# jalhajj/mahout

Measured on AMD Instinct MI355X. Metric: sketch updates/sec + item-pair cosines/sec @1M items, 1/2/4/8 MI355X, higher is better.
Workload: dtype u32

## Files before the change

mahout_amd/csrc/cms_api.hip:

```cpp
#include <hip/hip_runtime.h>

#include <atomic>
#include <chrono>
#include <rccl/rccl.h>

#include <algorithm>
#include <thread>
#include <cmath>
#include <cstdarg>
#include <cstdio>
#include <cstdlib>
#include <cstring>
#include <new>
#include <vector>

#include "cms_internal.h"

namespace cms {

static thread_local char g_err[512] = "";

int set_error(int code, const char* fmt, ...) {
  va_list ap;
  va_start(ap, fmt);
// ... 325 lines not shown
    if (hipGetDevice(&dev) != hipSuccess) dev = 0;
  }
  h->device = dev;
  hipError_t e = hipSetDevice(dev);
  if (e != hipSuccess) {
    delete h;
    return hip_fail(e, "hipSetDevice");
  }
  {
    int cus = 0;
    if (hipDeviceGetAttribute(&cus, hipDeviceAttributeMultiprocessorCount, dev) == hipSuccess && cus > 0)
      h->num_cus = cus;
  }
  h->n = p->num_owners;
  h->dw = (int64_t)p->depth * p->width;
  java_hash_params(p->seed, h->p.depth, h->a, h->b);
  HashParams& hp = h->hp;
  std::memset(&hp, 0, sizeof(hp));
  for (int i = 0; i < h->p.depth; ++i) {
    hp.ap[i] = reduce_key(h->a[i]);
    hp.bp[i] = reduce_key(h->b[i]);
  }
  hp.width = (uint32_t)h->p.width;
  hp.depth = h->p.depth;
  hp.frac_bits = p->frac_bits;
  hash_finish(hp);
  if (per_owner) h->dw = 0;

  size_t tbytes = sizeof(uint16_t) * (size_t)h->n * (size_t)h->dw;
  if ((e = hipStreamCreateWithFlags(&h->stream, hipStreamDefault)) != hipSuccess ||
      (e = hipStreamCreateWithFlags(&h->side_stream, hipStreamNonBlocking)) != hipSuccess ||
      (e = hipStreamCreateWithFlags(&h->side_stream2, hipStreamNonBlocking)) != hipSuccess ||
      (e = hipEventCreateWithFlags(&h->ev_join3, hipEventDisableTiming)) != hipSuccess ||
      (e = hipEventCreateWithFlags(&h->ev_spans, hipEventDisableTiming)) != hipSuccess ||
      (e = hipEventCreateWithFlags(&h->ev_plan, hipEventDisableTiming)) != hipSuccess ||
      (e = hipEventCreateWithFlags(&h->ev_fork2, hipEventDisableTiming)) != hipSuccess ||
      (e = hipEventCreateWithFlags(&h->ev_join2, hipEventDisableTiming)) != hipSuccess ||
#ifdef CMS_BUILD_GATHERHASH
      (e = hipMalloc((void**)&h->hp.gtab, sizeof(uint4) << 24)) != hipSuccess ||
#endif
      (!per_owner && !f64 && (e = hipMalloc(&h->d_off, sizeof(int64_t) * h->n)) != hipSuccess) ||
      (f64 && (e = hipMalloc(&h->d_t64, 4 * tbytes)) != hipSuccess) ||
      (!per_owner && (e = hipMalloc(&h->d_hidx, sizeof(int32_t) * h->n)) != hipSuccess) ||
      (!per_owner && (e = hipMemset(h->d_hidx, 0xff, sizeof(int32_t) * h->n)) != hipSuccess) ||
      (!per_owner && !f64 && (e = hipMalloc(&h->d_cbound, sizeof(uint32_t) * h->n)) != hipSuccess) ||
      (e = hipMalloc(&h->d_row_mass, sizeof(uint64_t) * h->n)) != hipSuccess ||
      (!per_owner && (e = hipMalloc(&h->d_norm, sizeof(uint64_t) * h->n * p->depth)) != hipSuccess) ||
      (!per_owner && (e = hipMalloc(&h->d_norm_sqrt, sizeof(double) * h->n * p->depth)) != hipSuccess) ||
      (e = hipMalloc(&h->d_rowmax, sizeof(uint32_t) * h->n)) != hipSuccess ||
      (e = hipMalloc(&h->d_flags, 64 * sizeof(uint32_t))) != hipSuccess ||
      (e = hipHostMalloc((void**)&h->h_pin, 16 * sizeof(uint32_t), hipHostMallocDefault)) != hipSuccess ||
      (e = hipMemset(h->d_flags, 0, 64 * sizeof(uint32_t))) != hipSuccess ||
      (e = hipMemset(h->d_row_mass, 0, sizeof(uint64_t) * h->n)) != hipSuccess) {
    int rc = hip_fail(e, "cms_create allocation");
    cms_destroy(h);
    return rc;
  }
  h->empty = true;
  h->norms_valid = false;
  h->forms_ok = !per_owner && !f64 && h->p.width % 32 == 0 && h->tune.forms;
  h->compact = h->forms_ok && !h->tune.no_compact &&
               (double)h->n * (double)(slot_units(h->dw) / kRowAlign + 1) < 4.0e9;
  if (!per_owner && !f64) {
    if (int rc = init_row_offsets(h)) {
      cms_destroy(h);
      return rc;
    }
  }
  *out = h;
  return CMS_OK;
}

int cms_create(const cms_params* p, cms_handle** out) { return create_impl(p, false, out); }

int cms_create_per_owner(const cms_params* p, cms_handle** out) { return create_impl(p, true, out); }

void cms_destroy(cms_handle* h) {
  if (!h) return;
  (void)hipSetDevice(h->device);
  if (h->stream) (void)hipStreamSynchronize(h->stream);
  for (auto& pe : h->pending) {
    (void)hipEventDestroy(pe.start);
    (void)hipEventDestroy(pe.stop);
  }
  for (hipEvent_t e : h->event_pool) (void)hipEventDestroy(e);
  if (h->order_ev) (void)hipEventDestroy(h->order_ev);
  if (h->side_stream) (void)hipStreamSynchronize(h->side_stream);
  if (h->side_stream2) (void)hipStreamSynchronize(h->side_stream2);
  if (h->ev_join3) (void)hipEventDestroy(h->ev_join3);
  if (h->ev_spans) (void)hipEventDestroy(h->ev_spans);
  if (h->ev_plan) (void)hipEventDestroy(h->ev_plan);
  if (h->ev_fork2) (void)hipEventDestroy(h->ev_fork2);
  if (h->ev_join2) (void)hipEventDestroy(h->ev_join2);
  free_query_pool(h);
  if (h->comm) (void)ncclCommDestroy(h->comm);
  arena_release(h);
  void* bufs[] = {h->d_off, h->d_t64, h->d_hidx, h->d_cbound, h->d_row_mass, h->d_norm, h->d_norm_sqrt, h->d_rowmax, h->d_flags, h->d_owner_ids};
  for (void* b : bufs)
    if (b) (void)hipFree(b);
  if (h->h_pin) (void)hipHostFree(h->h_pin);
  DevBuf* ws[] = {&h->ws_in_row, &h->ws_in_key, &h->ws_in_val, &h->ws_p1_row, &h->ws_p1_key, &h->ws_p1_val,
                  &h->ws_csr_key, &h->ws_csr_val, &h->ws_csr_off, &h->ws_csr_hi, &h->ws_hotpart, &h->ws_hist, &h->ws_small, &h->ws_partials,
                  &h->ws_hot, &h->ws_query, &h->ws_out, &h->ws_limb0, &h->ws_limbmeta, &h->ws_limbhot,
                  &h->ws_hotlist, &h->ws_tiles, &h->ws_slab, &h->ws_topq, &h->vl[0].buf, &h->vl[1].buf, &h->ws_nsq, &h->ws_cand,
                  &h->dlog_row, &h->dlog_key, &h->dlog_val, &h->dlog_cnt, &h->dlog_all, &h->ws_srow,
                  &h->ws_f4, &h->ws_i8blk, &h->po_off, &h->po_kp, &h->po_inc, &h->po_shape, &h->po_sk, &h->po_norm, &h->po_nsq,
                  &h->po_scratch, &h->po_wrows, &h->po_s0, &h->ws_pothr, &h->ws_posurv, &h->hot_tab, &h->ws_bound, &h->ws_force, &h->ws_plist, &h->ws_blist,
                  &h->ws_mbnd, &h->ws_mbits, &h->ws_mwoff, &h->ws_mpacked, &h->rf_ids, &h->rf_sc, &h->rf_cnt,
                  &h->rf_full, &h->rf_touch, &h->rf_new, &h->rf_redo, &h->rf_perm};
  for (DevBuf* b : ws) b->release();
  if (h->stream) (void)hipStreamDestroy(h->stream);
  if (h->side_stream) (void)hipStreamDestroy(h->side_stream);
  if (h->side_stream2) (void)hipStreamDestroy(h->side_stream2);
  delete h;
}

int cms_set_owner_ids(cms_handle* h, const int64_t* ids, int64_t n) {
  if (!h || !ids) return set_error(CMS_E_PARAM, "null argument");
  Guard g(h);
  if (n != h->n) return set_error(CMS_E_PARAM, "expected %lld owner IDs, got %lld", (long long)h->n, (long long)n);
  for (int64_t i = 1; i < n; ++i)
    if (ids[i] <= ids[i - 1]) return set_error(CMS_E_PARAM, "owner IDs must be strictly ascending");
// ... 1291 lines not shown
```

mahout_amd/csrc/cms_build.hip:

```cpp
#include <hip/hip_runtime.h>

#include <algorithm>
#include <cstdlib>

#include "cms_device.h"
#include "cms_internal.h"

namespace cms {

#ifdef CMS_BUILD_CHEAPHASH
#define bucket(hp, d, kp) ((uint32_t)(((kp) >> (d)) & (hp).wmask))
#endif
#ifdef CMS_BUILD_GATHERHASH
#define bucket(hp, d, kp) \
  ((uint32_t)(((&(hp).gtab[(kp) & 0xFFFFFFu].x)[((d) >> 1) & 3] >> (((d) & 1) << 4)) & (hp).wmask))
#endif

struct HotInfo {
  int64_t row;
  int32_t nslices;
  int32_t e0;
};

constexpr int kKeyRegs = 4;
// ... 388 lines not shown
    lds_barrier();
    d += two ? 2 : 1;
  }
  }

  if (badv) atomicOr(flags, kFlagBadValue);
  mass = wave_sum_u64_sat(mass);
  if ((tid & 63) == 0 && mass) atomicAdd(&s_mass, (unsigned long long)mass);
#pragma unroll
  for (int o = 32; o > 0; o >>= 1) vmax = max(vmax, (uint32_t)__shfl_xor((int)vmax, o, 64));
  if ((tid & 63) == 0 && vmax) atomicMax(&s_max, vmax);
  __syncthreads();
  if (!atomic_mode && tid < hp.depth) norm[row * hp.depth + tid] = s_norm[tid];
  if (!atomic_mode && tid == 0) rowmax[row] = s_max;
  if (tid == 0) {
    uint64_t tm = s_mass;
    if (!atomic_mode) {
      uint64_t m = accumulate ? row_mass[row] + tm : tm;
      row_mass[row] = m;
      if (m >= (1ULL << 32)) atomicOr(flags, kFlagOverflow);
    } else if (tm) {
      unsigned long long old = atomicAdd((unsigned long long*)&row_mass[row], (unsigned long long)tm);
      if (old + tm >= (1ULL << 32)) atomicOr(flags, kFlagOverflow);
    }
  }
}

constexpr int kMidThreads = 256;
constexpr int64_t kMidCachedKeys = (int64_t)kMidThreads * kKeyRegs;
constexpr int64_t kStreamBigKeys = 4096;
__device__ __forceinline__ int32_t list2_at(const int32_t* list, uint32_t cap, uint32_t nfront, uint32_t i) {
  return i < nfront ? list[i] : list[cap - 1u - (i - nfront)];
}
enum { kCntSlot = 0, kCntMid = 1 , kCntStream = 3 , kCntTicket = 5, kCntWords = 8 };
constexpr int kClassChunk = 4096;
__global__ __launch_bounds__(256) void k_build_classes(const int64_t* lo_, const int64_t* hi_, int64_t nrows,
                                                       const int32_t* hidx, const uint64_t* bound, int32_t* slot_list,
                                                       int32_t* mid_list, int32_t* stream_list, uint32_t* cnt) {
  __shared__ int32_t s_own[kClassChunk], s_str[kClassChunk];
  __shared__ uint32_t s_n[4], s_b[4];
  const int lane = (int)__lane_id();
  const int tid = threadIdx.x;
  const uint32_t cap = (uint32_t)nrows;
  const unsigned long long below = (1ULL << lane) - 1ULL;
  for (int64_t r0 = (int64_t)blockIdx.x * kClassChunk; r0 < nrows; r0 += (int64_t)gridDim.x * kClassChunk) {
    if (tid < 4) s_n[tid] = 0;
    __syncthreads();
    for (int64_t r = r0 + tid; r < r0 + kClassChunk; r += 256) {
      bool is[4] = {false, false, false, false};
      if (r < nrows) {
        const int32_t sl = hidx[r];
        const int64_t m = hi_[r] - lo_[r];
        is[0] = sl >= 0;
        const bool is_mid = !is[0] && !byte_class(sl, m, bound[r]);
        is[1] = is_mid && m <= kMidCachedKeys;
        is[2] = is_mid && m > kStreamBigKeys;
        is[3] = is_mid && !is[1] && !is[2];
      }
      unsigned long long mk[4];
      uint32_t b[4] = {0, 0, 0, 0};
#pragma unroll
      for (int k = 0; k < 4; ++k) {
        mk[k] = __ballot(is[k]);
        if (lane == 0 && mk[k]) b[k] = atomicAdd(&s_n[k], (uint32_t)__popcll(mk[k]));
        b[k] = (uint32_t)__shfl((int)b[k], 0, 64) + (uint32_t)__popcll(mk[k] & below);
      }
      if (is[0]) s_own[b[0]] = (int32_t)r;
      if (is[1]) s_own[kClassChunk - 1 - b[1]] = (int32_t)r;
      if (is[2]) s_str[b[2]] = (int32_t)r;
      if (is[3]) s_str[kClassChunk - 1 - b[3]] = (int32_t)r;
    }
    __syncthreads();
    if (tid < 4) {
      const int ci = tid == 0 ? kCntSlot : tid == 1 ? kCntMid + 1 : kCntStream + tid - 2;
      s_b[tid] = s_n[tid] ? atomicAdd(&cnt[ci], s_n[tid]) : 0u;
    }
    __syncthreads();
    for (uint32_t i = tid; i < s_n[0]; i += 256) slot_list[s_b[0] + i] = s_own[i];
    for (uint32_t i = tid; i < s_n[1]; i += 256) mid_list[cap - 1u - (s_b[1] + i)] = s_own[kClassChunk - 1 - i];
    for (uint32_t i = tid; i < s_n[2]; i += 256) stream_list[s_b[2] + i] = s_str[i];
    for (uint32_t i = tid; i < s_n[3]; i += 256) stream_list[cap - 1u - (s_b[3] + i)] = s_str[kClassChunk - 1 - i];
    __syncthreads();
  }
}

constexpr int kMidListKeys = kBuildThreads * kKeyRegs;
constexpr int kMidRowKeys = 4;
template <int SV, int D, int MT>
__device__ __forceinline__ void mid_rows(
    const int64_t* lo_, const int64_t* hi_, const Keys& keys, const float* vals, const HashParams& hp,
    const int32_t* list, const uint32_t* list_cnt, uint32_t cap, const TableView& tv, int32_t* hidx_w,
    uint32_t* cbound, uint64_t* row_mass, uint64_t* norm, uint32_t* rowmax, uint32_t* flags, int list_keys,
    int u4_keys, int u8_keys) {
  static_assert(MT == kMidThreads, "one instantiation per depth");
  constexpr int MTH = MT;
  constexpr int MKR = kKeyRegs;
  extern __shared__ __align__(16) uint32_t lds[];
  __shared__ unsigned long long s_norm[CMS_MAX_DEPTH];
  __shared__ unsigned long long s_mass;
  __shared__ uint32_t s_max, s_ovf;
  const int tid = threadIdx.x;
  const int w = (int)hp.width;
  const uint32_t nfront = list_cnt[0], count = nfront + list_cnt[1];
  for (uint32_t li = blockIdx.x; li < count; li += gridDim.x) {
    const int64_t row = list2_at(list, cap, nfront, li);
    const int64_t lo = lo_[row], hi = hi_[row];
    const bool cached = (hi - lo) <= (int64_t)MTH * MKR;
    uint64_t kp[MKR];
    uint32_t ik[MKR];
    uint64_t mass = 0;
    bool badv = false;
    if (cached) {
#pragma unroll
      for (int k = 0; k < MKR; ++k) {
        const int64_t i = lo + tid + (int64_t)k * MTH;
        kp[k] = 0;
        ik[k] = 0;
        if (i < hi) {
          uint32_t inc;
          if (!load_inc(vals, i, inc, hp.frac_bits)) {
            badv = true;
            inc = 0;
          }
          kp[k] = keys.at(i);
          ik[k] = inc;
          mass += inc;
        }
      }
    }
    uint4* d4 = reinterpret_cast<uint4*>(tv.row16(row));
    const int64_t m = hi - lo;
    const bool as_list = cached && m <= list_keys && vals == nullptr && hp.frac_bits == 0 &&
                         (int64_t)hp.depth * m <= 8192 && 2 + 2 * (int64_t)hp.depth * m < (int64_t)hp.depth * w / 2;
    uint16_t* lst = tv.row16(row);
    int level = -1;
    uint32_t vmax = 0;
    const int start = as_list || m <= u4_keys ? 0 : m <= u8_keys ? 1 : 2;
    bool mass_pending = !cached;
    if (start == 0) {
      constexpr int ab = 4;
      const int lga = 3;
      const uint32_t capa = (1u << ab) - 1u;
      const int nq_all = (int)((int64_t)hp.depth * w * ab >> 7);
      uint4* l4 = reinterpret_cast<uint4*>(lds);
      for (int j = tid; j < nq_all; j += MTH) l4[j] = make_uint4(0, 0, 0, 0);
      if (tid < CMS_MAX_DEPTH) s_norm[tid] = 0ULL;
      if (tid == 0) {
        s_max = 0u;
        s_ovf = 0u;
        s_mass = 0ULL;
      }
      __syncthreads();
      bool ovf = false;
      vmax = 0;
      constexpr int kSq = D > 0 ? D : 1;
      uint32_t sqr[kSq];
#pragma unroll
      for (int d = 0; d < kSq; ++d) sqr[d] = 0u;
      const bool tele = D > 0 && as_list;
      auto add_all = [&](uint64_t kr, uint32_t inc, int64_t lt) {
        each_bucket<D>(hp, kr, [&](int d, uint32_t bk) {
          if (lt >= 0) lst[1 + (int64_t)d * m + lt] = (uint16_t)bk;
          const uint32_t c = (uint32_t)d * (uint32_t)w + bk;
          const uint32_t sh = (c & ((1u << lga) - 1u)) * (uint32_t)ab;
          const uint32_t old = (atomicAdd(&lds[c >> lga], inc << sh) >> sh) & capa;
          const uint32_t nv = old + inc;
          ovf |= nv > capa || inc > capa;
          vmax = max(vmax, nv);
          if (D > 0) sqr[D > 0 ? d : 0] += (2u * old + inc) * inc;
        });
// ... 280 lines not shown
      if (tid < depth) {
        uint64_t s = 0;
#pragma unroll
        for (int k = 0; k < NW; ++k) s += red[k * RS + tid];
        norm[row * depth + tid] = s;
      }
      if (tid == 0) {
        rowmax[row] = mx;
        row_mass[row] = (uint64_t)m;
        hidx_w[row] = kFormU8;
        cbound[row] = mx;
      }
    }
    li = lds[0];
  }
}

template <int SV, int D, int MT>
__global__ __launch_bounds__(MT) __attribute__((amdgpu_waves_per_eu(MT == kStreamThreads ? 8 : 4, 8))) void k_build_mid(
    const int64_t* lo_, const int64_t* hi_, Keys keys, const float* vals, HashParams hp,
    const int32_t* list, const uint32_t* list_cnt , uint32_t cap, TableView tv, int32_t* hidx_w,
    uint32_t* cbound, uint64_t* row_mass, uint64_t* norm, uint32_t* rowmax, uint32_t* flags, int list_keys,
    int u4_keys, int u8_keys, int32_t* redo, uint32_t* redo_cnt, uint32_t* ticket) {
  if constexpr (MT == kStreamThreads)
    mid_streamed<SV, D>(lo_, hi_, keys, hp, list, list_cnt, cap, tv, hidx_w, cbound, row_mass, norm, rowmax, redo,
                        redo_cnt, ticket, u4_keys, u8_keys);
  else
    mid_rows<SV, D, MT>(lo_, hi_, keys, vals, hp, list, list_cnt, cap, tv, hidx_w, cbound, row_mass, norm, rowmax,
                        flags, list_keys, u4_keys, u8_keys);
}

constexpr int kMidGridPerCu = 8;
constexpr int kNibWaves = 4;
__host__ __device__ __forceinline__ int nib_first_bits(int64_t m, int w, int bit_keys, int crumb_keys) {
  return (m <= bit_keys && (w & 127) == 0) ? 1 : (m <= crumb_keys && (w & 63) == 0) ? 2 : 4;
}
__host__ __device__ __forceinline__ bool nib_list_row(int64_t m, int w, int d, bool weighted, int frac_bits,
                                                      int bit_keys, int crumb_keys, int list_keys) {
  return m <= list_keys && !weighted && frac_bits == 0 &&
         2 + 2 * (int64_t)d * m <= ((int64_t)d * w * nib_first_bits(m, w, bit_keys, crumb_keys)) / 8;
}

__global__ void k_row_caps(const int64_t* lo_, const int64_t* hi_, int64_t n, const uint64_t* bound,
                           const int32_t* hidx, int forms, int weighted, int frac_bits, int d, int w, int bit_keys,
                           int crumb_keys, int list_keys, uint32_t* caps) {
  const int64_t dw = (int64_t)d * w;
  const uint32_t full = (uint32_t)(slot_units(dw) / kRowAlign);
  for (int64_t r = blockIdx.x * (int64_t)blockDim.x + threadIdx.x; r < n; r += (int64_t)gridDim.x * blockDim.x) {
    const int32_t s = hidx[r];
    const int64_t m = hi_[r] - lo_[r];
    uint32_t c = full;
    if (s >= 0) {
      c = 0;
    } else if (forms && byte_class(s, m, bound[r])) {
      const int64_t u16s = nib_list_row(m, w, d, weighted != 0, frac_bits, bit_keys, crumb_keys, list_keys)
                               ? 1 + (int64_t)d * m
                               : dw / 2;
      c = (uint32_t)((u16s + kRowAlign - 1) / kRowAlign);
    }
    caps[r] = c;
  }
}

template <int SV>
__device__ __forceinline__ void nib_owner(
    int64_t row, uint32_t* lds, const int64_t* lo_, const int64_t* hi_, const Keys& keys, const float* vals,
    const HashParams& hp, const int32_t* row_hot, const uint64_t* bound, const TableView& tv, int32_t* hidx_w,
    uint32_t* cbound, uint64_t* row_mass, uint64_t* norm, uint32_t* rowmax, uint32_t* flags, int32_t* redo,
    uint32_t* redo_cnt, int bit_keys, int crumb_keys, int list_keys, int lists_done) {
  const int lane = threadIdx.x & 63;
  const int wv = threadIdx.x >> 6;
  const int64_t lo = lo_[row], hi = hi_[row];
  if (row_hot[row] >= 0 || !byte_class(tv.hidx[row], hi - lo, bound[row])) return;
  const int w = (int)hp.width;
// ... 233 lines not shown
      const int ns = (m + 63) >> 6;
      const bool ovf = ns == 1   ? list_rows<D, 1>(slot, pk, lane, m, sq, vmax)
                       : ns == 2 ? list_rows<D, 2>(slot, pk, lane, m, sq, vmax)
                       : ns == 3 ? list_rows<D, 3>(slot, pk, lane, m, sq, vmax)
                       : ns == 4 ? list_rows<D, 4>(slot, pk, lane, m, sq, vmax)
                                 : false;
      if (lane == 0) lst[0] = (uint16_t)m;
      if (ovf) {
        if (lane == 0) redo[atomicAdd(redo_cnt, 1u)] = ~(int32_t)row;
      } else {
#pragma unroll
        for (int q = 0; q < P; ++q) sq[q] = wave_fold_dpp(sq[q], [](uint32_t a, uint32_t b) { return a + b; });
        vmax = wave_fold_dpp(vmax, [](uint32_t a, uint32_t b) { return max(a, b); });
        if (lane < D) {
          uint32_t s = 0;
#pragma unroll
          for (int r = 0; r < D; ++r)
            if (lane == r) s = (sq[r >> 1] >> ((r & 1) << 4)) & 0xFFFFu;
          norm[row * D + lane] = s;
        }
        if (lane == 0) {
          rowmax[row] = vmax;
          row_mass[row] = (uint64_t)m;
          hidx_w[row] = kFormList;
          cbound[row] = vmax;
        }
      }
    }
    if (!more) break;
    row = nrow;
    lo = nlo;
    m = nm;
    raw0 = nraw0;
  }
}

template <int SV>
__global__ __launch_bounds__(kBuildThreads) void k_build_bytes(
    const int64_t* lo_, const int64_t* hi_, Keys keys, const float* vals, HashParams hp,
    const int32_t* list, const uint32_t* list_cnt, TableView tv, int32_t* hidx_w, uint32_t* cbound,
    uint64_t* row_mass, uint64_t* norm, uint32_t* rowmax, uint32_t* flags) {
  extern __shared__ __align__(16) uint32_t lds[];
  __shared__ unsigned long long s_norm[CMS_MAX_DEPTH];
  __shared__ uint32_t s_max, s_mass;
  const int tid = threadIdx.x;
  const int w = (int)hp.width;
  const int64_t dw = (int64_t)hp.depth * w;
  const uint32_t count = *list_cnt;
  for (uint32_t li = blockIdx.x; li < count; li += gridDim.x) {
    const bool keep_list = list[li] < 0;
    const int64_t row = keep_list ? ~(int64_t)list[li] : (int64_t)list[li];
    const int64_t lo = lo_[row], hi = hi_[row];
    uint16_t* lst = tv.row16(row);
    if (tid < CMS_MAX_DEPTH) s_norm[tid] = 0ULL;
    if (tid == 0) {
      s_max = 0u;
      s_mass = 0u;
    }
    uint64_t kp[kKeyRegs];
    uint32_t ik[kKeyRegs];
    uint32_t mass = 0;
    bool badv = false;
#pragma unroll
    for (int k = 0; k < kKeyRegs; ++k) {
      const int64_t i = lo + tid + (int64_t)k * kBuildThreads;
      kp[k] = 0;
// ... 301 lines not shown
  bool hot_norms_done = false;
  auto launch_hot_norms = [&]() -> int {
    TimedScope ts(h, "hot_norms");
    dim3 grid((unsigned)std::max<int64_t>(1, std::min<int64_t>(max_hot, 1024)), (unsigned)h->p.depth);
    hipLaunchKernelGGL(k_hot_norms, grid, dim3(256), 0, h->stream, hot, counters, h->hp, h->tview(), h->d_norm,
                       h->d_rowmax, whole_slices);
    CMS_HIP(hipGetLastError());
    hot_norms_done = true;
    return CMS_OK;
  };
  {
    TimedScope ts(h, "build_rows");
    auto kern = k_build_rows<kBuildStoreForm>;
    auto launch_slices = [&]() -> int {
      if (!fast_slices) return CMS_OK;
#ifdef CMS_BUILD_SKIP_SLICES
      return CMS_OK;
#endif
      static bool attr = [] {
        for (const void* f : {(const void*)k_build_slices<0>, (const void*)k_build_slices<4>,
                              (const void*)k_build_slices<5>})
          (void)hipFuncSetAttribute(f, hipFuncAttributeMaxDynamicSharedMemorySize, 80 * 1024);
        return true;
      }();
      (void)attr;
      auto kslices = h->p.depth == 5 ? k_build_slices<5> : h->p.depth == 4 ? k_build_slices<4> : k_build_slices<0>;
      hipLaunchKernelGGL(kslices, dim3((unsigned)emax), dim3(kSliceThreads), img_lds, h->stream, d_lo, d_hi,
                         keys, h->hp, kSliceKeys, hot, extra_map, counters, h->tview(), h->d_row_mass, h->d_flags,
                         whole_slices, h->d_norm, h->d_rowmax);
      CMS_HIP(hipGetLastError());
      return CMS_OK;
    };
    if (forms) {
      CMS_HIP(h->ws_blist.ensure(sizeof(int32_t) * (size_t)(3 * n + kCntWords)));
      int32_t* slot_list = h->ws_blist.as<int32_t>();
      int32_t* mid_list = slot_list + n;
      int32_t* stream_list = mid_list + n;
      uint32_t* lcnt = reinterpret_cast<uint32_t*>(stream_list + n);
      CMS_HIP(h->ws_plist.ensure(sizeof(int32_t) * (size_t)(n + 1)));
      int32_t* redo = h->ws_plist.as<int32_t>();
      uint32_t* redo_cnt = reinterpret_cast<uint32_t*>(redo + n);
      CMS_HIP(hipMemsetAsync(lcnt, 0, kCntWords * sizeof(uint32_t), h->stream));
      CMS_HIP(hipMemsetAsync(redo_cnt, 0, sizeof(uint32_t), h->stream));
      hipLaunchKernelGGL(k_build_classes,
                         dim3((unsigned)std::max<int64_t>(1, std::min<int64_t>((n + kClassChunk - 1) / kClassChunk, 1024))),
                         dim3(256), 0, h->stream, d_lo, d_hi, n, h->d_hidx, h->ws_bound.as<uint64_t>(), slot_list,
                         mid_list, stream_list, lcnt);
      CMS_HIP(hipGetLastError());
      if (h->plan_side_active) return set_error(CMS_E_STATE, "internal: side stream used while swapped for the plan");
      hipStream_t side = h->side_stream ? h->side_stream : h->stream;
#ifdef CMS_BUILD_SERIAL
      side = h->stream;
#endif
      const hipStream_t side2 = side != h->stream && h->tune.build_streams >= 3 ? h->side_stream2 : side;
      struct SideJoin {
        cms_handle* h;
        hipStream_t side, side2;
        bool armed = false;
        ~SideJoin() {
          if (armed && hipEventRecord(h->ev_join2, side) == hipSuccess)
            (void)hipStreamWaitEvent(h->stream, h->ev_join2, 0);
          if (armed && side2 != side && hipEventRecord(h->ev_join3, side2) == hipSuccess)
            (void)hipStreamWaitEvent(h->stream, h->ev_join3, 0);
        }
      } join{h, side, side2};
      if (side != h->stream) {
        CMS_HIP(hipEventRecord(h->ev_fork2, h->stream));
        CMS_HIP(hipStreamWaitEvent(side, h->ev_fork2, 0));
        if (side2 != side) CMS_HIP(hipStreamWaitEvent(side2, h->ev_fork2, 0));
        join.armed = true;
      }
      const int64_t nib_blocks = (n + kNibWaves - 1) / kNibWaves;
      const size_t nib_lds = (size_t)kNibWaves * (size_t)h->p.width / 2;
#if defined(CMS_BUILD_CHEAPHASH) || defined(CMS_BUILD_GATHERHASH)
      const int lists_done = 0;
#else
      const int lists_done = !d_val && h->hp.frac_bits == 0 && h->hp.fastq && lists_allowed(h) &&
                                     (h->p.depth == 4 || h->p.depth == 5)
                                 ? 1
                                 : 0;
#endif
      if (lists_done) {
        auto klists = h->p.depth == 5 ? k_build_lists<kBuildStoreForm, 5> : k_build_lists<kBuildStoreForm, 4>;
        if (h->lists_wgs_per_cu <= 0) {
          int per_cu = 0;
          CMS_HIP(hipOccupancyMaxActiveBlocksPerMultiprocessor(&per_cu, klists, 64 * kNibWaves, nib_lds));
          h->lists_wgs_per_cu = std::max(1, per_cu);
        }
        const int64_t lists_blocks = std::min<int64_t>(nib_blocks, (int64_t)h->num_cus * h->lists_wgs_per_cu);
        hipLaunchKernelGGL(klists, dim3((unsigned)lists_blocks), dim3(64 * kNibWaves), nib_lds, side, d_lo, d_hi, keys,
                           n, h->hp, row_hot, h->ws_bound.as<uint64_t>(), h->tview(), h->d_hidx, h->d_cbound,
                           h->d_row_mass, h->d_norm, h->d_rowmax, redo, redo_cnt, h->tune.bit_keys,
                           h->tune.crumb_keys, h->tune.list_keys);
      }
      bool nibbles_idle = lists_done != 0;
      for (int64_t m = 0; nibbles_idle && m < kByteKeys; ++m)
        nibbles_idle = nib_list_row(m, h->p.width, h->p.depth, false, 0, h->tune.bit_keys, h->tune.crumb_keys,
                                    h->tune.list_keys);
      if (!nibbles_idle)
        hipLaunchKernelGGL((k_build_nibbles<kBuildStoreForm, 0>), dim3((unsigned)nib_blocks), dim3(64 * kNibWaves),
                           nib_lds, side, d_lo, d_hi, keys, d_val, n, h->hp, row_hot, h->ws_bound.as<uint64_t>(),
                           h->tview(), h->d_hidx, h->d_cbound, h->d_row_mass, h->d_norm, h->d_rowmax, h->d_flags,
                           redo, redo_cnt, h->tune.bit_keys, h->tune.crumb_keys,
                           lists_allowed(h) ? h->tune.list_keys : 0, lists_done);
      const size_t mid_lds = std::max<size_t>((size_t)h->p.width * 2, (size_t)h->dw / 2);
      auto kmid = h->p.depth == 5   ? k_build_mid<kBuildStoreForm, 5, kMidThreads>
                  : h->p.depth == 4 ? k_build_mid<kBuildStoreForm, 4, kMidThreads>
                                    : k_build_mid<kBuildStoreForm, 0, kMidThreads>;
      auto launch_mid = [&](auto kern, int threads, unsigned grid, size_t klds, const int32_t* list, uint32_t* cnt) {
        hipLaunchKernelGGL(kern, dim3(grid), dim3(threads), klds, side2, d_lo, d_hi, keys, d_val, h->hp, list,
                           (const uint32_t*)cnt, (uint32_t)n, h->tview(), h->d_hidx, h->d_cbound, h->d_row_mass,
                           h->d_norm, h->d_rowmax, h->d_flags, lists_allowed(h) ? kMidListKeys : 0,
                           h->tune.mid_u4_keys, h->tune.mid_u8_keys, mid_list, lcnt + kCntMid, lcnt + kCntTicket);
      };
      const unsigned mid_grid = (unsigned)std::min<int64_t>(n, (int64_t)h->num_cus * kMidGridPerCu);
      bool one_pass = !d_val && h->hp.frac_bits == 0;
#ifdef CMS_BUILD_NO_STREAMED
      one_pass = false;
#endif
      if (one_pass) {
        auto kstr = h->p.depth == 5   ? k_build_mid<kBuildStoreForm, 5, kStreamThreads>
                    : h->p.depth == 4 ? k_build_mid<kBuildStoreForm, 4, kStreamThreads>
                                      : k_build_mid<kBuildStoreForm, 0, kStreamThreads>;
        const size_t str_lds = std::max<size_t>((size_t)h->dw, sizeof(uint32_t) * kStreamRedWords);
        if (h->stream_wgs_per_cu <= 0) {
          int per_cu = 0;
          CMS_HIP(hipOccupancyMaxActiveBlocksPerMultiprocessor(&per_cu, kstr, kStreamThreads, str_lds));
          h->stream_wgs_per_cu = std::max(1, per_cu);
        }
        launch_mid(kstr, kStreamThreads, (unsigned)std::min<int64_t>(n, (int64_t)h->num_cus * h->stream_wgs_per_cu),
                   str_lds, stream_list, lcnt + kCntStream);
      } else {
        launch_mid(kmid, kMidThreads, mid_grid, mid_lds, stream_list, lcnt + kCntStream);
      }
      launch_mid(kmid, kMidThreads, mid_grid, mid_lds, mid_list, lcnt + kCntMid);
      hipLaunchKernelGGL(k_build_bytes<kBuildStoreForm>, dim3((unsigned)std::min<int64_t>(n, (int64_t)h->num_cus * 2)),
                         dim3(kBuildThreads), (size_t)h->dw, side, d_lo, d_hi, keys, d_val, h->hp, redo, redo_cnt,
                         h->tview(), h->d_hidx, h->d_cbound, h->d_row_mass, h->d_norm, h->d_rowmax, h->d_flags);
      CMS_HIP(hipGetLastError());
      if ((rc0 = launch_slices())) return rc0;
      const int64_t nslot = std::min<int64_t>(n, h->hot_used);
      hipLaunchKernelGGL(kern, dim3((unsigned)(row_emax + nslot)), dim3(kBuildThreads), lds, h->stream, d_lo, d_hi,
                         keys, d_val, n, h->hp, kSliceKeys, row_hot, hot, extra_map, counters, row_emax, h->tview(),
                         h->d_row_mass, h->d_norm, h->d_rowmax, h->d_flags, accumulate, slices_done,
                         h->ws_bound.as<uint64_t>(), forms, skip_untouched, h->d_hidx, h->d_cbound,
                         (const int32_t*)slot_list, (const uint32_t*)lcnt);
      CMS_HIP(hipGetLastError());
      if (join.armed) {
        join.armed = false;
        CMS_HIP(hipEventRecord(h->ev_join2, side));
        CMS_HIP(hipStreamWaitEvent(h->stream, h->ev_join2, 0));
        if (side2 != side) {
          CMS_HIP(hipEventRecord(h->ev_join3, side2));
          CMS_HIP(hipStreamWaitEvent(h->stream, h->ev_join3, 0));
        }
      }
    } else {
      if ((rc0 = launch_slices())) return rc0;
      hipLaunchKernelGGL(kern, dim3((unsigned)(row_emax + n)), dim3(kBuildThreads), lds, h->stream, d_lo, d_hi, keys,
                         d_val, n, h->hp, kSliceKeys, row_hot, hot, extra_map, counters, row_emax, h->tview(),
                         h->d_row_mass, h->d_norm, h->d_rowmax, h->d_flags, accumulate, slices_done,
                         h->ws_bound.as<uint64_t>(), forms, skip_untouched, h->d_hidx, h->d_cbound,
                         (const int32_t*)nullptr, (const uint32_t*)nullptr);
      CMS_HIP(hipGetLastError());
    }
  }
  if (!hot_norms_done && (rc0 = launch_hot_norms())) return rc0;
// ... 7 lines not shown
```

mahout_amd/csrc/cms_internal.h:

```cpp
#pragma once
#include <hip/hip_runtime.h>
#include <rccl/rccl.h>

#include <functional>
#include <map>
#include <mutex>
#include <shared_mutex>
#include <string>
#include <vector>

#include "../../include/mahout_cms.h"
#include "cms_forms.h"
#include "cms_hash.h"

namespace cms {

enum : uint32_t {
  kFlagBadRow = 1u << 0,
  kFlagBadValue = 1u << 1,
  kFlagOverflow = 1u << 2,
};

struct DevBuf {
  void* ptr = nullptr;
// ... 125 lines not shown
}

namespace cms {
struct Tunables {
  int bit_keys = 64;
  int crumb_keys = 256;
  int list_keys = 256;
  int mid_u4_keys = 768;
  int mid_u8_keys = 12288;
  int plan_side = 1;
  int build_streams = 3;
  int po_dense_x4 = 4;
  int po_bound_part2 = 1;
  int po_bound_rows = 1;
  int po_no_prune = 0;
  int po_no_bigq = 0;
  int split_keys = 0;
  bool forms = true;
  bool no_compact = false;
  bool no_vmm = false;
  bool hot_routing = true;
  bool fp4 = true;
  bool mls = true;
};
}

struct cms_handle {
  cms_params p{};
  cms::Tunables tune;
  int device = 0;
  int num_cus = 256;
  int stream_wgs_per_cu = 0;
  int lists_wgs_per_cu = 0;
  hipStream_t stream = nullptr;
  hipStream_t side_stream = nullptr;
  hipEvent_t ev_fork2 = nullptr, ev_join2 = nullptr;
  hipStream_t side_stream2 = nullptr;
  hipEvent_t ev_join3 = nullptr;
  hipEvent_t ev_spans = nullptr, ev_plan = nullptr;
  bool spans_event = false, plan_side_request = false;
  bool plan_side_active = false;
  std::shared_mutex mu;
  std::mutex pool_mu;
  std::vector<cms::QueryCtx*> qpool;

  int64_t a[CMS_MAX_DEPTH] = {};
  int64_t b[CMS_MAX_DEPTH] = {};
  cms::HashParams hp{};

  int64_t n = 0;
  int64_t dw = 0;
  uint16_t* d_t16 = nullptr;
  int64_t t16_cap = 0, t16_used = 0;
  int64_t* d_off = nullptr;
  struct ArenaChunk {
    hipMemGenericAllocationHandle_t mem;
    size_t bytes;
  };
  void* arena_va = nullptr;
  size_t arena_va_bytes = 0, arena_mapped = 0, arena_gran = 0;
  int arena_small_layouts = 0;
  std::vector<ArenaChunk> arena_chunks;
  bool compact = false;
  bool f64 = false;
  double* d_t64 = nullptr;
  int32_t* d_hidx = nullptr;
  uint32_t* d_cbound = nullptr;
  bool forms_ok = false;
  cms::DevBuf hot_tab;
  cms::DevBuf ws_bound, ws_force, ws_plist;
  cms::DevBuf ws_blist;
// ... 308 lines not shown
```

Baseline: 55.67 billion.

## Route cached mid rows eligible for list form to a dedicated wave-per-row kernel

Adds a fifth class to the row classifier that picks cached mid rows qualifying for the compact list form. These rows go to a new k_build_mid_lists kernel on the side stream, which hashes keys in registers, counts collisions through a per-wave LDS slot array and writes list entries plus norms directly. Rows that overflow are pushed back onto the mid list for the generic path, with an event added so the later mid launch waits for them. The aim is to take the list-eligible rows off the heavier generic mid kernel, at the cost of an extra launch, a cross-stream dependency and more classifier LDS.

```diff
diff --git a/mahout_amd/csrc/cms_api.hip b/mahout_amd/csrc/cms_api.hip
--- a/mahout_amd/csrc/cms_api.hip
+++ b/mahout_amd/csrc/cms_api.hip
@@ -381,6 +381,7 @@
       (e = hipStreamCreateWithFlags(&h->side_stream, hipStreamNonBlocking)) != hipSuccess ||
       (e = hipStreamCreateWithFlags(&h->side_stream2, hipStreamNonBlocking)) != hipSuccess ||
       (e = hipEventCreateWithFlags(&h->ev_join3, hipEventDisableTiming)) != hipSuccess ||
+      (e = hipEventCreateWithFlags(&h->ev_mid_lists, hipEventDisableTiming)) != hipSuccess ||
       (e = hipEventCreateWithFlags(&h->ev_spans, hipEventDisableTiming)) != hipSuccess ||
       (e = hipEventCreateWithFlags(&h->ev_plan, hipEventDisableTiming)) != hipSuccess ||
       (e = hipEventCreateWithFlags(&h->ev_fork2, hipEventDisableTiming)) != hipSuccess ||
@@ -437,6 +438,7 @@
   if (h->side_stream) (void)hipStreamSynchronize(h->side_stream);
   if (h->side_stream2) (void)hipStreamSynchronize(h->side_stream2);
   if (h->ev_join3) (void)hipEventDestroy(h->ev_join3);
+  if (h->ev_mid_lists) (void)hipEventDestroy(h->ev_mid_lists);
   if (h->ev_spans) (void)hipEventDestroy(h->ev_spans);
   if (h->ev_plan) (void)hipEventDestroy(h->ev_plan);
   if (h->ev_fork2) (void)hipEventDestroy(h->ev_fork2);
diff --git a/mahout_amd/csrc/cms_build.hip b/mahout_amd/csrc/cms_build.hip
--- a/mahout_amd/csrc/cms_build.hip
+++ b/mahout_amd/csrc/cms_build.hip
@@ -444,35 +444,58 @@
 __device__ __forceinline__ int32_t list2_at(const int32_t* list, uint32_t cap, uint32_t nfront, uint32_t i) {
   return i < nfront ? list[i] : list[cap - 1u - (i - nfront)];
 }
-enum { kCntSlot = 0, kCntMid = 1 , kCntStream = 3 , kCntTicket = 5, kCntWords = 8 };
+__host__ __device__ __forceinline__ int nib_first_bits(int64_t m, int w, int bit_keys, int crumb_keys) {
+  return (m <= bit_keys && (w & 127) == 0) ? 1 : (m <= crumb_keys && (w & 63) == 0) ? 2 : 4;
+}
+__host__ __device__ __forceinline__ bool nib_list_row(int64_t m, int w, int d, bool weighted, int frac_bits,
+                                                      int bit_keys, int crumb_keys, int list_keys) {
+  return m <= list_keys && !weighted && frac_bits == 0 &&
+         2 + 2 * (int64_t)d * m <= ((int64_t)d * w * nib_first_bits(m, w, bit_keys, crumb_keys)) / 8;
+}
+__host__ __device__ __forceinline__ bool mid_list_row(int64_t m, int w, int d, bool weighted, int frac_bits,
+                                                      int list_keys) {
+  return m <= list_keys && !weighted && frac_bits == 0 && (int64_t)d * m <= 8192 &&
+         2 + 2 * (int64_t)d * m < (int64_t)d * w / 2;
+}
+enum {
+  kCntSlot = 0,
+  kCntMid = 1 ,
+  kCntStream = 3 ,
+  kCntTicket = 5,
+  kCntMidLists = 6,
+  kCntWords = 8
+};
 constexpr int kClassChunk = 4096;
 __global__ __launch_bounds__(256) void k_build_classes(const int64_t* lo_, const int64_t* hi_, int64_t nrows,
                                                        const int32_t* hidx, const uint64_t* bound, int32_t* slot_list,
-                                                       int32_t* mid_list, int32_t* stream_list, uint32_t* cnt) {
-  __shared__ int32_t s_own[kClassChunk], s_str[kClassChunk];
-  __shared__ uint32_t s_n[4], s_b[4];
+                                                       int32_t* mid_list, int32_t* stream_list, uint32_t* cnt,
+                                                       int32_t* mid_lists, int mid_lists_keys, int d, int w) {
+  __shared__ int32_t s_own[kClassChunk], s_str[kClassChunk], s_lst[kClassChunk];
+  __shared__ uint32_t s_n[5], s_b[5];
   const int lane = (int)__lane_id();
   const int tid = threadIdx.x;
   const uint32_t cap = (uint32_t)nrows;
   const unsigned long long below = (1ULL << lane) - 1ULL;
   for (int64_t r0 = (int64_t)blockIdx.x * kClassChunk; r0 < nrows; r0 += (int64_t)gridDim.x * kClassChunk) {
-    if (tid < 4) s_n[tid] = 0;
+    if (tid < 5) s_n[tid] = 0;
     __syncthreads();
     for (int64_t r = r0 + tid; r < r0 + kClassChunk; r += 256) {
-      bool is[4] = {false, false, false, false};
+      bool is[5] = {false, false, false, false, false};
       if (r < nrows) {
         const int32_t sl = hidx[r];
         const int64_t m = hi_[r] - lo_[r];
         is[0] = sl >= 0;
         const bool is_mid = !is[0] && !byte_class(sl, m, bound[r]);
-        is[1] = is_mid && m <= kMidCachedKeys;
+        const bool cached = is_mid && m <= kMidCachedKeys;
+        is[4] = cached && mid_list_row(m, w, d, false, 0, mid_lists_keys);
+        is[1] = cached && !is[4];
         is[2] = is_mid && m > kStreamBigKeys;
-        is[3] = is_mid && !is[1] && !is[2];
-      }
-      unsigned long long mk[4];
-      uint32_t b[4] = {0, 0, 0, 0};
-#pragma unroll
-      for (int k = 0; k < 4; ++k) {
+        is[3] = is_mid && !cached && !is[2];
+      }
+      unsigned long long mk[5];
+      uint32_t b[5] = {0, 0, 0, 0, 0};
+#pragma unroll
+      for (int k = 0; k < 5; ++k) {
         mk[k] = __ballot(is[k]);
         if (lane == 0 && mk[k]) b[k] = atomicAdd(&s_n[k], (uint32_t)__popcll(mk[k]));
         b[k] = (uint32_t)__shfl((int)b[k], 0, 64) + (uint32_t)__popcll(mk[k] & below);
@@ -481,10 +504,11 @@
       if (is[1]) s_own[kClassChunk - 1 - b[1]] = (int32_t)r;
       if (is[2]) s_str[b[2]] = (int32_t)r;
       if (is[3]) s_str[kClassChunk - 1 - b[3]] = (int32_t)r;
+      if (is[4]) s_lst[b[4]] = (int32_t)r;
     }
     __syncthreads();
-    if (tid < 4) {
-      const int ci = tid == 0 ? kCntSlot : tid == 1 ? kCntMid + 1 : kCntStream + tid - 2;
+    if (tid < 5) {
+      const int ci = tid == 0 ? kCntSlot : tid == 1 ? kCntMid + 1 : tid == 4 ? kCntMidLists : kCntStream + tid - 2;
       s_b[tid] = s_n[tid] ? atomicAdd(&cnt[ci], s_n[tid]) : 0u;
     }
     __syncthreads();
@@ -492,6 +516,7 @@
     for (uint32_t i = tid; i < s_n[1]; i += 256) mid_list[cap - 1u - (s_b[1] + i)] = s_own[kClassChunk - 1 - i];
     for (uint32_t i = tid; i < s_n[2]; i += 256) stream_list[s_b[2] + i] = s_str[i];
     for (uint32_t i = tid; i < s_n[3]; i += 256) stream_list[cap - 1u - (s_b[3] + i)] = s_str[kClassChunk - 1 - i];
+    for (uint32_t i = tid; i < s_n[4]; i += 256) mid_lists[s_b[4] + i] = s_lst[i];
     __syncthreads();
   }
 }
@@ -542,12 +567,11 @@
     }
     uint4* d4 = reinterpret_cast<uint4*>(tv.row16(row));
     const int64_t m = hi - lo;
-    const bool as_list = cached && m <= list_keys && vals == nullptr && hp.frac_bits == 0 &&
-                         (int64_t)hp.depth * m <= 8192 && 2 + 2 * (int64_t)hp.depth * m < (int64_t)hp.depth * w / 2;
+    const bool as_list = cached && mid_list_row(m, w, hp.depth, vals != nullptr, hp.frac_bits, list_keys);
     uint16_t* lst = tv.row16(row);
     int level = -1;
     uint32_t vmax = 0;
-    const int start = as_list || m <= u4_keys ? 0 : m <= u8_keys ? 1 : 2;
+    const int start = cached && li < nfront ? 2 : as_list || m <= u4_keys ? 0 : m <= u8_keys ? 1 : 2;
     bool mass_pending = !cached;
     if (start == 0) {
       constexpr int ab = 4;
@@ -894,14 +918,6 @@
 
 constexpr int kMidGridPerCu = 8;
 constexpr int kNibWaves = 4;
-__host__ __device__ __forceinline__ int nib_first_bits(int64_t m, int w, int bit_keys, int crumb_keys) {
-  return (m <= bit_keys && (w & 127) == 0) ? 1 : (m <= crumb_keys && (w & 63) == 0) ? 2 : 4;
-}
-__host__ __device__ __forceinline__ bool nib_list_row(int64_t m, int w, int d, bool weighted, int frac_bits,
-                                                      int bit_keys, int crumb_keys, int list_keys) {
-  return m <= list_keys && !weighted && frac_bits == 0 &&
-         2 + 2 * (int64_t)d * m <= ((int64_t)d * w * nib_first_bits(m, w, bit_keys, crumb_keys)) / 8;
-}
 
 __global__ void k_row_caps(const int64_t* lo_, const int64_t* hi_, int64_t n, const uint64_t* bound,
                            const int32_t* hidx, int forms, int weighted, int frac_bits, int d, int w, int bit_keys,
@@ -1201,6 +1217,195 @@
     lo = nlo;
     m = nm;
     raw0 = nraw0;
+  }
+}
+
+constexpr int kMidListWaves = 4;
+constexpr int kMidListSlots = 16;
+constexpr int kMidListGroup = 4;
+constexpr int kMidListSlotMax = 8192;
+static_assert(64 * kMidListSlots == kMidListKeys && kMidListSlots % kMidListGroup == 0, "every cached list row fits");
+
+template <int D>
+__device__ __forceinline__ bool mid_list_rows(uint32_t* slot, const uint32_t (&pk)[kMidListSlots][(D + 1) / 2],
+                                              uint32_t live, int ns, uint32_t (&sq)[D], uint32_t& vmax) {
+  bool ovf = false;
+#pragma unroll
+  for (int r = 0; r < D; ++r) {
+    uint32_t old[kMidListSlots];
+#pragma unroll
+    for (int k = 0; k < kMidListSlots; ++k)
+      if (k < ns) {
+        const uint32_t c = (pk[k][r >> 1] >> ((r & 1) << 4)) & 0xFFFFu;
+        old[k] = atomicAdd(&slot[c >> 2], ((live >> k) & 1u) << ((c & 3u) << 3));
+      }
+#pragma unroll
+    for (int k = 0; k < kMidListSlots; ++k)
+      if (k < ns) {
+        uint32_t p = pk[k][r >> 1];
+        asm volatile("" : "+v"(p));
+        const uint32_t c = (p >> ((r & 1) << 4)) & 0xFFFFu;
+        const uint32_t lv = (live >> k) & 1u;
+        const uint32_t o = (old[k] >> ((c & 3u) << 3)) & 255u;
+        const uint32_t nv = (o + 1u) * lv;
+        ovf |= nv > 255u;
+        sq[r] += (2u * o + 1u) * lv;
+        vmax = max(vmax, nv);
+        slot[c >> 2] = 0u;
+      }
+    if (__ballot(ovf)) return true;
+  }
+  return false;
+}
+
+template <int SV, int D>
+__global__ __launch_bounds__(64 * kMidListWaves) __attribute__((amdgpu_waves_per_eu(4, 8))) void k_build_mid_lists(
+    const int64_t* lo_, const int64_t* hi_, Keys keys, HashParams hp, const int32_t* list, const uint32_t* list_cnt,
+    TableView tv, int32_t* hidx_w, uint32_t* cbound, uint64_t* row_mass, uint64_t* norm, uint32_t* rowmax,
+    int32_t* redo, uint32_t* redo_cnt) {
+  extern __shared__ __align__(16) uint32_t lds[];
+  constexpr int P = (D + 1) / 2;
+  constexpr int NSL = kMidListSlots, GS = kMidListGroup, NGR = NSL / GS;
+  const int lane = threadIdx.x & 63;
+  const int wv = __builtin_amdgcn_readfirstlane(threadIdx.x >> 6);
+  const int w = (int)hp.width;
+  uint32_t* slot = lds + wv * (w >> 2);
+  for (int j = lane; j < (w >> 2); j += 64) slot[j] = 0u;
+  const uint32_t count = list_cnt[0];
+  const uint32_t idle = ((4u * (uint32_t)lane) & hp.wmask) * 0x10001u;
+  double qa[D], qb[D];
+  uint32_t am[D], bm[D];
+#pragma unroll
+  for (int r = 0; r < D; ++r) {
+    qa[r] = hp.qa[r];
+    qb[r] = hp.qb[r];
+    am[r] = (uint32_t)hp.ap[r] & hp.wmask;
+    bm[r] = (uint32_t)hp.bp[r];
+  }
+  const uint32_t stride = gridDim.x * kMidListWaves;
+  const uint32_t li = blockIdx.x * kMidListWaves + wv;
+  if (li >= count) return;
+  int32_t row = list[li];
+  int32_t row1 = li + stride < count ? list[li + stride] : -1;
+  uint32_t li2 = li + 2u * stride;
+  int64_t lo = lo_[row];
+  int m = (int)(hi_[row] - lo);
+  int64_t base = tv.base(row);
+  uint64_t raw0 = lane < m ? keys.raw(lo + lane) : 0ULL;
+  for (;;) {
+    const int32_t row2 = li2 < count ? list[li2] : -1;
+    li2 += stride;
+    int64_t nlo = 0, nhi = 0, nbase = 0;
+    if (row1 >= 0) {
+      nlo = lo_[row1];
+      nhi = hi_[row1];
+      nbase = tv.base(row1);
+    }
+    uint16_t* lst = tv.t16 + base;
+    uint32_t pk[NSL][P];
+    {
+      uint64_t cur[GS], nxt[GS];
+      cur[0] = raw0;
+#pragma unroll
+      for (int j = 1; j < GS; ++j) cur[j] = lane + 64 * j < m ? keys.raw(lo + lane + 64 * j) : 0ULL;
+#pragma unroll
+      for (int g = 0; g < NGR; ++g) {
+#pragma unroll
+        for (int j = 0; j < GS; ++j) nxt[j] = 0ULL;
+        if (g + 1 < NGR && 64 * GS * (g + 1) < m) {
+#pragma unroll
+          for (int j = 0; j < GS; ++j) {
+            const int t = lane + 64 * (GS * (g + 1) + j);
+            if (t < m) nxt[j] = keys.raw(lo + t);
+          }
+        }
+#pragma unroll
+        for (int j = 0; j < GS; ++j)
+#pragma unroll
+          for (int q = 0; q < P; ++q) pk[GS * g + j][q] = idle;
+        if (64 * GS * g < m) {
+#pragma unroll
+          for (int j = 0; j < GS; ++j) {
+            const int k = GS * g + j;
+            if (lane + 64 * k < m) {
+              uint16_t* e = lst + 1 + lane + 64 * k;
+              const uint64_t kp = keys.resolve(cur[j]);
+              const double kf = (double)(uint32_t)kp;
+              const uint32_t km = (uint32_t)kp & hp.wmask;
+              bool redo_key = (kp >> 32) != 0;
+#pragma unroll
+              for (int q = 0; q < P; ++q) pk[k][q] = 0u;
+#pragma unroll
+              for (int r = 0; r < D; ++r) {
+                const double y = fma(qa[r], kf, qb[r]);
+                const double fl = floor(y);
+                const double fr = y - fl;
+                redo_key |= !(fr >= kQEps && fr <= 1.0 - kQEps);
+                const uint32_t q = (uint32_t)__double_as_longlong(fl + 4503599627370496.0);
+                const uint32_t c = (__umul24(am[r], km) + bm[r] + __umul24(q, 25u)) & hp.wmask;
+                e[r * m] = (uint16_t)c;
+                pk[k][r >> 1] |= c << ((r & 1) << 4);
+              }
+              if (redo_key) {
+#pragma unroll 1
+                for (int r = 0; r < D; ++r) {
+                  const uint32_t c = bucket(hp, r, kp);
+                  e[r * m] = (uint16_t)c;
+#pragma unroll
+                  for (int q = 0; q < P; ++q)
+                    if ((r >> 1) == q)
+                      pk[k][q] = (r & 1) ? (pk[k][q] & 0xFFFFu) | (c << 16) : (pk[k][q] & 0xFFFF0000u) | c;
+                }
+              }
+            }
+          }
+        }
+#pragma unroll
+        for (int j = 0; j < GS; ++j) cur[j] = nxt[j];
+      }
+    }
+    int nm = 0;
+    uint64_t nraw0 = 0ULL;
+    if (row1 >= 0) {
+      nm = (int)(nhi - nlo);
+      if (lane < nm) nraw0 = keys.raw(nlo + lane);
+    }
+    uint32_t sq[D];
+#pragma unroll
+    for (int r = 0; r < D; ++r) sq[r] = 0u;
+    uint32_t vmax = 0;
+    const int nf = min(max((m - lane + 63) >> 6, 0), NSL);
+    const uint32_t live = (1u << nf) - 1u;
+    const int ns = (m + 63) >> 6;
+    const bool ovf = mid_list_rows<D>(slot, pk, live, ns, sq, vmax);
+    if (ovf) {
+      if (lane == 0) redo[atomicAdd(redo_cnt, 1u)] = row;
+    } else {
+#pragma unroll
+      for (int r = 0; r < D; ++r) sq[r] = wave_fold_dpp(sq[r], [](uint32_t a, uint32_t b) { return a + b; });
+      vmax = wave_fold_dpp(vmax, [](uint32_t a, uint32_t b) { return max(a, b); });
+      if (lane < D) {
+        uint32_t s = 0;
+#pragma unroll
+        for (int r = 0; r < D; ++r)
+          if (lane == r) s = sq[r];
+        norm[(int64_t)row * D + lane] = s;
+      }
+      if (lane == 0) {
+        lst[0] = (uint16_t)m;
+        rowmax[row] = vmax;
+        row_mass[row] = (uint64_t)m;
+        hidx_w[row] = kFormList;
+        cbound[row] = vmax;
+      }
+    }
+    if (row1 < 0) break;
+    row = row1;
+    lo = nlo;
+    m = nm;
+    base = nbase;
+    raw0 = nraw0;
+    row1 = row2;
   }
 }
 
@@ -1568,20 +1773,31 @@
       return CMS_OK;
     };
     if (forms) {
-      CMS_HIP(h->ws_blist.ensure(sizeof(int32_t) * (size_t)(3 * n + kCntWords)));
+      CMS_HIP(h->ws_blist.ensure(sizeof(int32_t) * (size_t)(4 * n + kCntWords)));
       int32_t* slot_list = h->ws_blist.as<int32_t>();
       int32_t* mid_list = slot_list + n;
       int32_t* stream_list = mid_list + n;
-      uint32_t* lcnt = reinterpret_cast<uint32_t*>(stream_list + n);
+      int32_t* mid_lists = stream_list + n;
+      uint32_t* lcnt = reinterpret_cast<uint32_t*>(mid_lists + n);
       CMS_HIP(h->ws_plist.ensure(sizeof(int32_t) * (size_t)(n + 1)));
       int32_t* redo = h->ws_plist.as<int32_t>();
       uint32_t* redo_cnt = reinterpret_cast<uint32_t*>(redo + n);
+#if defined(CMS_BUILD_CHEAPHASH) || defined(CMS_BUILD_GATHERHASH)
+      const int lists_done = 0;
+#else
+      const int lists_done = !d_val && h->hp.frac_bits == 0 && h->hp.fastq && lists_allowed(h) &&
+                                     (h->p.depth == 4 || h->p.depth == 5)
+                                 ? 1
+                                 : 0;
+#endif
+      const bool mid_lists_done = lists_done && h->p.width <= kMidListSlotMax;
       CMS_HIP(hipMemsetAsync(lcnt, 0, kCntWords * sizeof(uint32_t), h->stream));
       CMS_HIP(hipMemsetAsync(redo_cnt, 0, sizeof(uint32_t), h->stream));
       hipLaunchKernelGGL(k_build_classes,
                          dim3((unsigned)std::max<int64_t>(1, std::min<int64_t>((n + kClassChunk - 1) / kClassChunk, 1024))),
                          dim3(256), 0, h->stream, d_lo, d_hi, n, h->d_hidx, h->ws_bound.as<uint64_t>(), slot_list,
-                         mid_list, stream_list, lcnt);
+                         mid_list, stream_list, lcnt, mid_lists, mid_lists_done ? kMidListKeys : 0, h->p.depth,
+                         h->p.width);
       CMS_HIP(hipGetLastError());
       if (h->plan_side_active) return set_error(CMS_E_STATE, "internal: side stream used while swapped for the plan");
       hipStream_t side = h->side_stream ? h->side_stream : h->stream;
@@ -1608,14 +1824,22 @@
       }
       const int64_t nib_blocks = (n + kNibWaves - 1) / kNibWaves;
       const size_t nib_lds = (size_t)kNibWaves * (size_t)h->p.width / 2;
-#if defined(CMS_BUILD_CHEAPHASH) || defined(CMS_BUILD_GATHERHASH)
-      const int lists_done = 0;
-#else
-      const int lists_done = !d_val && h->hp.frac_bits == 0 && h->hp.fastq && lists_allowed(h) &&
-                                     (h->p.depth == 4 || h->p.depth == 5)
-                                 ? 1
-                                 : 0;
-#endif
+      if (mid_lists_done) {
+        auto kml = h->p.depth == 5 ? k_build_mid_lists<kBuildStoreForm, 5> : k_build_mid_lists<kBuildStoreForm, 4>;
+        const size_t ml_lds = (size_t)kMidListWaves * (size_t)h->p.width;
+        if (h->mid_lists_wgs_per_cu <= 0) {
+          int per_cu = 0;
+          CMS_HIP(hipOccupancyMaxActiveBlocksPerMultiprocessor(&per_cu, kml, 64 * kMidListWaves, ml_lds));
+          h->mid_lists_wgs_per_cu = std::max(1, per_cu);
+        }
+        const int64_t ml_blocks = std::min<int64_t>((n + kMidListWaves - 1) / kMidListWaves,
+                                                    (int64_t)h->num_cus * h->mid_lists_wgs_per_cu);
+        hipLaunchKernelGGL(kml, dim3((unsigned)ml_blocks), dim3(64 * kMidListWaves), ml_lds, side, d_lo, d_hi, keys,
+                           h->hp, (const int32_t*)mid_lists, (const uint32_t*)(lcnt + kCntMidLists), h->tview(),
+                           h->d_hidx, h->d_cbound, h->d_row_mass, h->d_norm, h->d_rowmax, mid_list, lcnt + kCntMid);
+        CMS_HIP(hipGetLastError());
+        if (side2 != side) CMS_HIP(hipEventRecord(h->ev_mid_lists, side));
+      }
       if (lists_done) {
         auto klists = h->p.depth == 5 ? k_build_lists<kBuildStoreForm, 5> : k_build_lists<kBuildStoreForm, 4>;
         if (h->lists_wgs_per_cu <= 0) {
@@ -1669,6 +1893,7 @@
       } else {
         launch_mid(kmid, kMidThreads, mid_grid, mid_lds, stream_list, lcnt + kCntStream);
       }
+      if (mid_lists_done && side2 != side) CMS_HIP(hipStreamWaitEvent(side2, h->ev_mid_lists, 0));
       launch_mid(kmid, kMidThreads, mid_grid, mid_lds, mid_list, lcnt + kCntMid);
       hipLaunchKernelGGL(k_build_bytes<kBuildStoreForm>, dim3((unsigned)std::min<int64_t>(n, (int64_t)h->num_cus * 2)),
                          dim3(kBuildThreads), (size_t)h->dw, side, d_lo, d_hi, keys, d_val, h->hp, redo, redo_cnt,
diff --git a/mahout_amd/csrc/cms_internal.h b/mahout_amd/csrc/cms_internal.h
--- a/mahout_amd/csrc/cms_internal.h
+++ b/mahout_amd/csrc/cms_internal.h
@@ -181,11 +181,13 @@
   int num_cus = 256;
   int stream_wgs_per_cu = 0;
   int lists_wgs_per_cu = 0;
+  int mid_lists_wgs_per_cu = 0;
   hipStream_t stream = nullptr;
   hipStream_t side_stream = nullptr;
   hipEvent_t ev_fork2 = nullptr, ev_join2 = nullptr;
   hipStream_t side_stream2 = nullptr;
   hipEvent_t ev_join3 = nullptr;
+  hipEvent_t ev_mid_lists = nullptr;
   hipEvent_t ev_spans = nullptr, ev_plan = nullptr;
   bool spans_event = false, plan_side_request = false;
   bool plan_side_active = false;
```

After: 59.21 billion, median of 6. +6.4%, better.
